# Totoketchup/Adaptive-MultiSpeaker-Separation

Hardware: AMD Instinct MI355X
Metric: mixtures/sec training throughput (2-spk, 256-filter adapt+BLSTM-DPCL) (higher is better)
Workload: dtype f32 (storage, accumulation and results f32; dense products issued on the 16-bit matrix pipe as fp16x3 / bf16x6 emulation of the f32 product -- `value_native_f32` is the same step on v_mfma_f32_32x32x2_f32)

## Files before the change

### adaptive-multispeaker-separation_amd/ams_hip/_lib.py

```python
import ctypes
import os
import re

_HERE = os.path.dirname(os.path.abspath(__file__))
LIB_PATH = os.environ.get('AMS_HIP_LIB') or os.path.join(_HERE, 'libams_hip.so')
HEADER_PATH = os.path.normpath(os.path.join(_HERE, '..', '..', 'include', 'ams.h'))

ABI_VERSION = 5

_CT = {
    'int': ctypes.c_int, 'long': ctypes.c_long, 'float': ctypes.c_float, 'size_t': ctypes.c_size_t,
    'int32_t': ctypes.c_int32, 'ams_status': ctypes.c_int32, 'void': None,
}


def parse_header(path=HEADER_PATH):
    src = open(path).read()
    src = re.sub(r'/\*.*?\*/', ' ', src, flags=re.S)
    protos = {}
    for m in re.finditer(r'\b(ams_status|size_t|int|long|void)\s+(ams_\w+)\s*\(([^)]*)\)\s*;', src):
        ret, name, args = m.group(1), m.group(2), m.group(3).strip()
        argtypes = []
        if args and args != 'void':
            for a in args.split(','):
# ... 50 lines not shown
```

### adaptive-multispeaker-separation_amd/ams_hip/functional.py

```python
import torch
from torch.autograd import Function

from . import ops


def _c(t):
    return t if t.is_contiguous() else t.contiguous()


class _Overlap(object):

    def __init__(self):
        self.enabled = False
        self.stream = None
        self.n_cap = 0
        self.deferred = []
        self.on_ready = None

    def side(self):
        if self.stream is None:
            import os
            self.stream = torch.cuda.Stream(priority=int(os.environ.get('AMS_SIDE_PRIORITY', '0')))
        return self.stream

# ... 205 lines not shown
        return ops.dense_fwd(x, W, b, amax=ctx.amax)

    @staticmethod
    def backward(ctx, du):
        x, W = ctx.saved_tensors
        du2 = _c(du).view(-1, W.shape[1])
        x2 = x.reshape(-1, x.shape[-1])
        b = ctx.bias
        am_dx = am_dw = None
        if ctx.amax is not None:
            adu = ops.amax_of(du2)
            am_dx, am_dw = (adu, ctx.amax[1]), (ctx.amax[0], adu)
        if OVERLAP.usable(W, b) and ctx.needs_input_grad[1] and ctx.needs_input_grad[2]:
            dx = None
            if _DENSE_MODE == 0 and _ORDER >= 1 and ctx.needs_input_grad[0]:
                dx = ops.gemm(du2, W, transB=True, amax=am_dx).view(x.shape)
            s = OVERLAP.fork(x2, du2)
            Nw = W.shape[1]
            cuts = _dw_cuts(Nw) if (_DENSE_MODE == 0 and ctx.needs_input_grad[0] and W.grad.stride(0) == Nw) else [(0, Nw)]

            def piece(n0, n1):
                Wg = W.grad if (n0, n1) == (0, Nw) else W.grad[:, n0:n1]
                dus = du2 if (n0, n1) == (0, Nw) else du2[:, n0:n1]
                with OVERLAP.capped('dense', _DENSE_MODE == 0):
                    fused = ops.gemm_at_b_colsum(x2, dus, Wg, b.grad[n0:n1], accumulate=True, amax=am_dw, ldc=W.grad.stride(0))
                    if not fused:
                        ops.gemm(x2, dus, transA=True, out=Wg, accumulate=True, amax=am_dw, M=x2.shape[1], N=n1 - n0, K=x2.shape[0],
                                 lda=x2.stride(0), ldb=du2.stride(0), ldc=W.grad.stride(0))
                if not fused:
                    ops.colsum_into(_c(dus), b.grad[n0:n1], True)
            with torch.cuda.stream(s):
                piece(*cuts[0])
            for i, c in enumerate(cuts[1:]):
                last = i == len(cuts) - 2
                OVERLAP.defer(lambda c=c, last=last: (piece(*c), OVERLAP.ready(W, b) if last else None))
            if len(cuts) == 1:
                OVERLAP.ready(W, b)
            if _DENSE_MODE == 2 and ctx.needs_input_grad[0]:
                torch.cuda.current_stream().wait_stream(s)
            if dx is None and ctx.needs_input_grad[0]:
                dx = ops.gemm(du2, W, transB=True, amax=am_dx).view(x.shape)
            return dx, None, None
        dx = ops.gemm(du2, W, transB=True, amax=am_dx).view(x.shape) if ctx.needs_input_grad[0] else None
        dW = ops.gemm(x2, du2, transA=True, amax=am_dw) if ctx.needs_input_grad[1] else None
        db = ops.colsum(du2) if ctx.needs_input_grad[2] else None
        return dx, dW, db


class L2Norm(Function):

    @staticmethod
    def forward(ctx, u, E):
        v, inv = ops.l2norm_fwd(u, E)
        ctx.save_for_backward(v, inv)
        ctx.E = E
        return v.view(u.shape[:-1] + (u.shape[-1] // E, E))

    @staticmethod
# ... 637 lines not shown
```

### adaptive-multispeaker-separation_amd/ams_hip/ops.py

```python
import ctypes
import os as _os

import torch

from ._lib import load, check, AmsError

_vp = ctypes.c_void_p


def _p(t):
    return _vp(t.data_ptr()) if t is not None else _vp(0)


def _s():
    return _vp(torch.cuda.current_stream().cuda_stream)


def _chk(*ts):
    for t in ts:
        if t is None:
            continue
        if not t.is_cuda:
            raise AmsError('ams_hip ops need device tensors (there is no CPU fallback)')
        if t.dtype != torch.float32 or not t.is_contiguous():
# ... 186 lines not shown
        a = getattr(b, '_ams_amax', None)
        if a is not None and a[1] == b._version:
            return a[0]
        b = b._base
    return absmax(t)


PASS = [0]


def _frozen(*ts):
    return all(getattr(t, '_ams_frozen', False) for t in ts)


def drop_frozen_derivatives(t):
    for k in ('_ams_amax_cache', '_ams_wcat', '_ams_wcat_amax', '_ams_kbound', '_ams_bcat', '_ams_ps_w'):
        if hasattr(t, k):
            delattr(t, k)


class _ParamSource(object):
    __slots__ = ('flat', 'bound', 'seen', 'event', 'used', 'next', 'rolled', '__weakref__')

    def __init__(self, flat):
        self.flat = flat
        self.bound = torch.zeros(1, dtype=torch.float32, device=flat.device)
        self.next = torch.zeros(192, dtype=torch.int32, device=flat.device)
        self.rolled = False
        self.seen = -1
        self.event = None
        self.used = -1
# ... 388 lines not shown
            and (bias is None or bias.data_ptr() % 16 == 0) and max(M, N) * ((K + 31) // 32 * 128) < 2 ** 31
            and load().ams_gemm_get_arith() != 0)


def forward_product(x2, W2, bias, out, amax, label, owner, ldc=None):
    M, K = x2.shape
    N = W2.shape[1]
    ldc = (out.stride(0) if out.dim() == 2 else N) if ldc is None else ldc
    if not (forward_product_presplit(M, N, K, out, bias, amax, label, ldc) and x2.stride(1) == 1 and W2.stride(1) == 1):
        return gemm(x2, W2, bias=bias, out=out, M=M, N=N, K=K, lda=x2.stride(0), ldb=W2.stride(0), ldc=ldc, label=label, amax=amax)
    a_img = ps_pack_rows(x2, amax[0])
    b_img = _ps_weight_image(W2, amax[1], owner)
    return gemm_ps(a_img, b_img, K, amax, bias=bias, out=out, ldc=ldc, label=label)


def gemm_at_b_colsum(A, B, out, bsum, accumulate=True, amax=None, ldc=None):
    K, M = A.shape
    N = B.shape[1]
    ldc = out.stride(0) if ldc is None else ldc
    ok = (M % 4 == 0 and N % 4 == 0 and A.stride(0) % 4 == 0 and B.stride(0) % 4 == 0 and A.stride(1) == 1 and B.stride(1) == 1
          and out.stride(-1) == 1 and bsum.stride(-1) == 1 and bsum.data_ptr() % 16 == 0
          and all(t.data_ptr() % 16 == 0 for t in (A, B)) and _os.environ.get('AMS_GEMM_NOVEC') is None)
    if not ok:
        return False
    lib = load()
    pad = LDS_PAD[0]
    nb = lib.ams_gemm_workspace_bytes(M, N, K, 1, pad)
    ws = _ws(nb, A) if nb else None
    bws = _ws(32 * N * 4, A)
    ev = PROFILE.begin() if PROFILE.enabled else None
# ... 266 lines not shown
    dx = None
    if need_dx:
        dxf = gemm(dZ, Kf, transB=True, M=M, N=D, K=4 * H, lda=8 * H, ldb=ldu, ldc=D,
                   out=torch.empty((M, D), dtype=torch.float32, device=x.device))
        dxb = gemm(dZ[4 * H:], Kb, transB=True, M=M, N=D, K=4 * H, lda=8 * H, ldb=ldu, ldc=D,
                   out=torch.empty((M, D), dtype=torch.float32, device=x.device))
        dx = dxf.view(B, T, D) * masks['in'][0] + dxb.view(B, T, D) * masks['in'][1]
    return dx, dKf, dbf, dKb, dbb


def blstm_bwd_dx(G, Kf, Kb, B, T, D, amax=None):
    H = Kf.shape[1] // 4
    M = B * T
    Wcat = blstm_wcat(Kf, Kb, D)
    dx = torch.empty((B, T, D), dtype=torch.float32, device=G.device)
    gemm(G.view(-1), Wcat, transB=True, out=dx, M=M, N=D, K=8 * H, lda=8 * H, ldb=8 * H, ldc=D, amax=amax)
    return dx


def blstm_bwd_weights(x, out, G, dKf, dbf, dKb, dbb, accumulate, part='all', dbpart=None, amax=None):
    lib = load()
    am_wx = (amax[0], amax[2]) if amax is not None else None
    am_u = (amax[1], amax[2]) if amax is not None else None
    B, T, D = x.shape
    H = dKf.shape[1] // 4
    M = B * T
    x2 = x.view(M, D)
    dZf = G.view(-1)
    dZb = G.view(-1)[4 * H:]
    acc = bool(accumulate)
    _chk_rows(dKf, dKb)
# ... 648 lines not shown
```

### adaptive-multispeaker-separation_amd/csrc/common.h

```cpp
#pragma once
#include <hip/hip_runtime.h>
#include <stdint.h>
#include <stddef.h>
#include "../../include/ams.h"

typedef float f32x4 __attribute__((ext_vector_type(4)));
typedef float f32x16 __attribute__((ext_vector_type(16)));

extern thread_local int g_ams_last_hip_error;

static inline ams_status ams_check_launch() {
    hipError_t e = hipGetLastError();
    if (e != hipSuccess) {
        g_ams_last_hip_error = (int)e;
        return AMS_E_LAUNCH_FAILED;
    }
    return AMS_OK;
}

#define AMS_REQUIRE(cond)            \
    do {                             \
        if (!(cond)) return AMS_E_INVALID_ARG; \
    } while (0)

static inline int ceil_div(long a, long b) { return (int)((a + b - 1) / b); }

namespace ams_detail {
size_t conv_maxpool_ps_bytes(int Bt, int L, int W, int N);
bool conv_maxpool_ps_applies(int Bt, int L, int W, int N);
ams_status conv_maxpool_ps(const float* x, const float* f, float* pmax, int32_t* pidx, int Bt, int L, int W, int N, int pl,
                           const float* amax_x, const float* amax_f, void* img, hipStream_t st);
}

__device__ __forceinline__ float wave_sum(float v) {
#pragma unroll
    for (int o = 32; o > 0; o >>= 1) v += __shfl_xor(v, o, 64);
    return v;
}
template <int S>
__device__ __forceinline__ float lane_above(float v) {
    const unsigned b = __builtin_bit_cast(unsigned, v);
    if constexpr (S == 32 || S == 16) {
        unsigned hi = b, lo = 0u;
        if constexpr (S == 32) asm volatile("s_nop 1\n\tv_permlane32_swap_b32 %0, %1\n\ts_nop 1" : "+v"(hi), "+v"(lo));
        else asm volatile("s_nop 1\n\tv_permlane16_swap_b32 %0, %1\n\ts_nop 1" : "+v"(hi), "+v"(lo));
        return __builtin_bit_cast(float, lo);
// ... 25 lines not shown
```

### adaptive-multispeaker-separation_amd/csrc/gemm.hip

```cpp
#include "common.h"
#include <stdlib.h>
#include <atomic>
#include <type_traits>

namespace {

struct LaunchOpt { const float* amax_a = nullptr; const float* amax_b = nullptr; int lds_pad = 0; void* sk_scratch = nullptr; size_t sk_bytes = 0;
                   unsigned* amax_out = nullptr; int force_cfg = -1; };
constexpr size_t AMS_SK_FLAG_BYTES = 8192;
constexpr size_t AMS_SK_SLOT_BYTES = (128 * 256 + 256) * sizeof(float);
std::atomic<int> g_gemm_arith{-1};

struct GemmTuning { int group_m, splits, x6cfg, x6rule, x6persist, sk; bool noprio, novec, f16x3; double x6waste; bool c_vec; };
inline const GemmTuning& tuning() {
    static const GemmTuning t = [] {
        GemmTuning v{0, 0, -1, 2, 1, 1, false, false, true, 1.30, true};
        if (const char* f = getenv("AMS_GEMM_CVEC")) v.c_vec = atoi(f) != 0;
        if (const char* f = getenv("AMS_GEMM_SK")) v.sk = atoi(f);
        if (const char* f = getenv("AMS_GEMM_X6WASTE")) v.x6waste = atof(f);
        if (const char* f = getenv("AMS_GEMM_GROUP_M")) v.group_m = atoi(f);
        if (const char* f = getenv("AMS_GEMM_SPLITS")) v.splits = atoi(f);
        v.noprio = getenv("AMS_GEMM_NOPRIO") != nullptr;
        { const char* e = getenv("AMS_X6_PERSIST"); v.x6persist = e ? atoi(e) : 1; }
        { const char* e = getenv("AMS_GEMM_F16X3"); v.f16x3 = !(e && atoi(e) == 0); }
// ... 1361 lines not shown
            if (blocks > 2048) blocks = 2048;
            hipLaunchKernelGGL(splitk_reduce_kernel, dim3(blocks, nbatch), dim3(256), 0, st, g.partial, g.C, g.bias, g.M, g.N, g.ldc,
                               splits, g.accumulate, g.c_zs, g.bias_zs);
        }
        s = ams_check_launch();
    }
    if (s == AMS_OK && bsum_out && !bsum_in_launch) {
        if (!vec || BMODE != B_ROW) return AMS_E_INVALID_ARG;
        hipLaunchKernelGGL(bsum_finish_kernel, dim3(ceil_div(g.N, 256)), dim3(256), 0, st, bsum_ws, bsum_out, g.N, splits, bsum_accumulate);
        s = ams_check_launch();
    }
    return s;
}

inline bool aligned16(const void* p) { return ((uintptr_t)p & 15) == 0; }

}

extern "C" {

void ams_gemm_set_arith(int mode) { g_gemm_arith.store(mode ? 1 : 0, std::memory_order_relaxed); }
int ams_gemm_get_arith(void) { return use_x6() ? 1 : 0; }

size_t ams_gemm_sk_scratch_bytes(void) {
    const size_t g8 = (size_t)(device_cus() + 7) / 8 * 8;
    const size_t a = g8 * 2 * (128 * 128 + 128) * sizeof(float), b = g8 * AMS_SK_SLOT_BYTES;
    return AMS_SK_FLAG_BYTES + (a > b ? a : b);
}

size_t ams_gemm_workspace_bytes(int M, int N, int K, int nbatch, int lds_pad) {
// ... 625 lines not shown
```

### adaptive-multispeaker-separation_amd/csrc/gemm_ps.hip

```cpp
#include "common.h"
#include <type_traits>

namespace {

typedef _Float16 f16x8_t __attribute__((ext_vector_type(8)));
typedef _Float16 f16x2_t __attribute__((ext_vector_type(2)));
typedef float f32x2_t __attribute__((ext_vector_type(2)));
typedef __attribute__((address_space(3))) void lds_void;
typedef int i32x4_t __attribute__((ext_vector_type(4)));

constexpr int PS_BK = 32, PS_BM = 128, PS_BN = 256, PS_NT = 512;
constexpr int PS_A_BYTES = PS_BM * 128, PS_B_BYTES = PS_BN * 128, PS_STAGE = PS_A_BYTES + PS_B_BYTES;
constexpr int PS_STAGES = 3;
constexpr int PS_BIAS_OFF = PS_STAGES * PS_STAGE;
constexpr int PS_LDS = PS_BIAS_OFF + 2 * 1024;

__device__ __forceinline__ unsigned ps_pk_f16(float a, float b) {
    const f32x2_t v = {a, b};
    return __builtin_bit_cast(unsigned, __builtin_convertvector(v, f16x2_t));
}
__device__ __forceinline__ void ps_split2(float a, float b, unsigned& hi, unsigned& lo) {
    hi = ps_pk_f16(a, b);
    const f16x2_t h = __builtin_bit_cast(f16x2_t, hi);
    lo = ps_pk_f16(a - (float)h[0], b - (float)h[1]);
// ... 90 lines not shown
    ps_split2(v[6] * s, v[7] * s, hi.w, lo.w);
    unsigned char* p = img + (((long)c * R + sgn) * lpp + t) * 32;
    *reinterpret_cast<uint4*>(p) = hi;
    *reinterpret_cast<uint4*>(p + 16) = lo;
}

struct PsArgs {
    const unsigned char* A; const unsigned char* B; float* C; const float* bias;
    const float* amax_a; const float* amax_b;
    int M, N, K;
    long ldc;
    unsigned pitch_a, pitch_b;
    int tiles_m, tiles_n, group_m;
    int conv_L, conv_R; unsigned conv_lpp; long a_bytes;
    int32_t* pidx;
};

__device__ __forceinline__ void ps_locate(const PsArgs& g, int item, int& tile_m, int& tile_n) {
    const int items = g.tiles_m * g.tiles_n;
    const int q = items / 8, r = items % 8, xcd = item % 8, idx = item / 8;
    const int bid = (xcd < r ? xcd * (q + 1) : r * (q + 1) + (xcd - r) * q) + idx;
    const int gm = g.group_m > 0 ? g.group_m : 1;
    const int band = bid / (gm * g.tiles_n), within = bid - band * (gm * g.tiles_n);
    const int band_rows = min(gm, g.tiles_m - band * gm);
    tile_n = within / band_rows;
    tile_m = band * gm + (within - tile_n * band_rows);
}

#ifndef AMS_PS_SLEEP
#define AMS_PS_SLEEP 0
#endif
#ifndef AMS_PS_STAMP
#define AMS_PS_STAMP 0
#endif
#if AMS_PS_STAMP
__device__ long long g_ps_stamp[1024 * 8 * 8];
#define PS_STAMP(ph) do { if (threadIdx.x == 0 && wi < 8) g_ps_stamp[((int)blockIdx.x * 8 + wi) * 8 + (ph)] = wall_clock64(); } while (0)
#else
#define PS_STAMP(ph) do { } while (0)
#endif

template <bool CONV>
__global__ __launch_bounds__(PS_NT, 1) void gemm_ps_kernel(const PsArgs g) {
    extern __shared__ __attribute__((aligned(1024))) unsigned char ps_smem[];
    const int tid = threadIdx.x, lane = tid & 63;
    const int wave = __builtin_amdgcn_readfirstlane(tid >> 6);
    const int wm = wave >> 2, wn = wave & 3;
    const int l31 = lane & 31, lk = lane >> 5;
    const int nk = (g.K + PS_BK - 1) / PS_BK;
    const int n_items = g.tiles_m * g.tiles_n, G = (int)gridDim.x;
    const int n_work = (n_items - (int)blockIdx.x + G - 1) / G;
    if (n_work <= 0) return;
    __builtin_amdgcn_s_setprio(2);

    auto rsrc = [](const unsigned char* p, long bytes) {
        const unsigned long long a = (unsigned long long)(uintptr_t)p;
        i32x4_t r = {(int)(unsigned)a, (int)(unsigned)((a >> 32) & 0xffffu), (int)bytes, 0x00020000};
        r.x = __builtin_amdgcn_readfirstlane(r.x); r.y = __builtin_amdgcn_readfirstlane(r.y);
        r.z = __builtin_amdgcn_readfirstlane(r.z); r.w = __builtin_amdgcn_readfirstlane(r.w);
        return r;
    };
    const i32x4_t rsA = rsrc(g.A, CONV ? g.a_bytes : (long)g.M * g.pitch_a), rsB = rsrc(g.B, (long)g.N * g.pitch_b);
    const i32x4_t rsBias = rsrc(reinterpret_cast<const unsigned char*>(g.bias), g.bias ? (long)g.N * 4 : 0);

    const int drow = lane >> 3, dslot = lane & 7;
    const int f_even = (drow >> 1) & 7, f_odd = (4 + (drow >> 1)) & 7;
    const unsigned pa_even = (unsigned)(dslot ^ f_even) * 16u, pa_odd = (unsigned)(dslot ^ f_odd) * 16u;
    unsigned voffA[2], voffB[4];

    const int ff = (l31 >> 1) & 7;
    unsigned fa[2], fb[2];
#pragma unroll
    for (int i = 0; i < 2; ++i) {
        if constexpr (CONV)
            fa[i] = (unsigned)((wm * 64 + 8 * (l31 & 7) + 4 * i + (l31 >> 3)) * 128 + ((lk ^ (l31 & 7)) * 16));
        else
            fa[i] = (unsigned)(((wm * 2 + i) * 32 + l31) * 128 + ((lk ^ ff) * 16));
    }
#pragma unroll
    for (int j = 0; j < 2; ++j) fb[j] = (unsigned)(PS_A_BYTES + ((wn * 2 + j) * 32 + l31) * 128 + ((lk ^ ff) * 16));

    const float sc_inv = (1.0f / ps_scale(g.amax_a[0])) * (1.0f / ps_scale(g.amax_b[0]));

    int tile_m, tile_n, m0, n0;
    auto setup = [&](int i) {
        ps_locate(g, (int)blockIdx.x + i * G, tile_m, tile_n);
        m0 = tile_m * PS_BM; n0 = tile_n * PS_BN;
        if constexpr (CONV) {
            const int sgn = m0 / g.conv_L, pb = m0 - sgn * g.conv_L;
#pragma unroll
            for (int q = 0; q < 2; ++q) {
                const int A_ = 2 * wave + q, a = A_ & 7, row = (A_ >> 3) * 64 + 8 * drow + a;
                const int p = pb + row;
                const unsigned pc = (unsigned)(dslot ^ a);
                const unsigned off = ((((unsigned)a * (unsigned)g.conv_R + (unsigned)sgn) * g.conv_lpp + (unsigned)(p >> 3) + (pc & 3u)) * 2u + (pc >> 2)) * 16u;
                voffA[q] = (m0 + row < g.M) ? off : 0xfffffff0u;
            }
        } else {
#pragma unroll
            for (int q = 0; q < 2; ++q) voffA[q] = (unsigned)(m0 + (2 * wave + q) * 8 + drow) * g.pitch_a + (q ? pa_odd : pa_even);
        }
#pragma unroll
        for (int q = 0; q < 4; ++q) voffB[q] = (unsigned)(n0 + (4 * wave + q) * 8 + drow) * g.pitch_b + ((q & 1) ? pa_odd : pa_even);
    };
    const unsigned lds0 = (unsigned)(uintptr_t)(lds_void*)ps_smem;
    auto issue1 = [&](int kt, int stage, int q) {
        const bool isA = q < 2;
        const unsigned ld = lds0 + (unsigned)(stage * PS_STAGE + (isA ? (2 * wave + q) * 1024 : PS_A_BYTES + (4 * wave + q - 2) * 1024));
        const unsigned vo = isA ? voffA[q] : voffB[q - 2];
        const int ko = kt * 128;
        unsigned keep;
        if (isA)
            asm volatile("s_mov_b32 %0, m0\n\ts_mov_b32 m0, %1\n\ts_nop 0\n\tbuffer_load_dwordx4 %2, %3, %4 offen lds\n\ts_mov_b32 m0, %0"
                         : "=&s"(keep) : "s"(ld), "v"(vo), "s"(rsA), "s"(ko) : "memory");
        else
            asm volatile("s_mov_b32 %0, m0\n\ts_mov_b32 m0, %1\n\ts_nop 0\n\tbuffer_load_dwordx4 %2, %3, %4 offen lds\n\ts_mov_b32 m0, %0"
                         : "=&s"(keep) : "s"(ld), "v"(vo), "s"(rsB), "s"(ko) : "memory");
    };
    auto issue = [&](int kt, int stage) {
#pragma unroll
        for (int q = 0; q < 6; ++q) issue1(kt, stage, q);
    };

    auto issue_bias = [&](int par) {
        if (wave == 0) {
            const unsigned lb = lds0 + (unsigned)(PS_BIAS_OFF + par * 1024);
            const unsigned vo = (unsigned)(n0 * 4 + lane * 16);
            unsigned keep;
            asm volatile("s_mov_b32 %0, m0\n\ts_mov_b32 m0, %1\n\ts_nop 0\n\tbuffer_load_dwordx4 %2, %3, 0 offen lds\n\ts_mov_b32 m0, %0"
                         : "=&s"(keep) : "s"(lb), "v"(vo), "s"(rsBias) : "memory");
        }
    };

    f32x16 acc[2][2], accs[2][2];
    f16x8_t carry[2][2];
    bool prime = true;
    auto frags = [&](const unsigned char* sb, int ks, f16x8_t (&a)[2][2], f16x8_t (&b)[2][2]) {
#pragma unroll
        for (int i = 0; i < 2; ++i)
#pragma unroll
// ... 3 lines not shown
            }
#pragma unroll
        for (int j = 0; j < 2; ++j)
#pragma unroll
            for (int p = 0; p < 2; ++p) b[j][p] = *reinterpret_cast<const f16x8_t*>(sb + (fb[j] ^ (unsigned)(ks * 32 + p * 64)));
    };
    auto four = [&](f32x16 (&c)[2][2], const f16x8_t (&a)[2][2], const f16x8_t (&b)[2][2], int pa, int pb) {
#pragma unroll
        for (int i = 0; i < 2; ++i)
#pragma unroll
            for (int j = 0; j < 2; ++j) c[i][j] = __builtin_amdgcn_mfma_f32_32x32x16_f16(a[i][pa], b[j][pb], c[i][j], 0, 0, 0);
#if AMS_PS_SLEEP
        __builtin_amdgcn_s_sleep(AMS_PS_SLEEP);
#endif
    };
    auto mfma_tile = [&](int stage, auto PRE, int kt2, int stage2) {
        constexpr bool pre = decltype(PRE)::value;
        const unsigned char* const sb = ps_smem + stage * PS_STAGE;
        f16x8_t a0[2][2], b0[2][2], a1[2][2], b1[2][2];
        if constexpr (CONV) {
            if (prime) {
#pragma unroll
                for (int ks = 0; ks < 2; ++ks)
#pragma unroll
                    for (int p = 0; p < 2; ++p) carry[ks][p] = *reinterpret_cast<const f16x8_t*>(sb + (fa[0] ^ (unsigned)(ks * 32 + p * 64)));
                prime = false;
            }
        }
        frags(sb, 0, a0, b0);
        __builtin_amdgcn_sched_barrier(0);
        four(accs, a0, b0, 1, 0);
        __builtin_amdgcn_sched_barrier(0);
        if constexpr (pre) issue1(kt2, stage2, 0);
        frags(sb, 1, a1, b1);
        __builtin_amdgcn_sched_barrier(0);
        four(accs, a0, b0, 0, 1);
        __builtin_amdgcn_sched_barrier(0);
        if constexpr (pre) issue1(kt2, stage2, 1);
        __builtin_amdgcn_sched_barrier(0);
        four(acc, a0, b0, 0, 0);
        __builtin_amdgcn_sched_barrier(0);
        if constexpr (pre) issue1(kt2, stage2, 2);
        __builtin_amdgcn_sched_barrier(0);
        four(accs, a1, b1, 1, 0);
        __builtin_amdgcn_sched_barrier(0);
        if constexpr (pre) issue1(kt2, stage2, 3);
        __builtin_amdgcn_sched_barrier(0);
        four(accs, a1, b1, 0, 1);
        __builtin_amdgcn_sched_barrier(0);
        if constexpr (pre) { issue1(kt2, stage2, 4); issue1(kt2, stage2, 5); }
        __builtin_amdgcn_sched_barrier(0);
        four(acc, a1, b1, 0, 0);
        if constexpr (CONV) {
#pragma unroll
            for (int p = 0; p < 2; ++p) { carry[0][p] = a0[1][p]; carry[1][p] = a1[1][p]; }
        }
    };

    setup(0);
    issue(0, 0);
    issue_bias(0);
    if (nk > 1) issue(1, 1);
    for (int wi = 0; wi < n_work; ++wi) {
        PS_STAMP(0);
#pragma unroll
        for (int i = 0; i < 2; ++i)
#pragma unroll
            for (int j = 0; j < 2; ++j)
#pragma unroll
                for (int r = 0; r < 16; ++r) { acc[i][j][r] = 0.f; accs[i][j][r] = 0.f; }
        prime = true;
        int st = 0;
        for (int kt = 0; kt < nk - 2; ++kt) {
            asm volatile("s_waitcnt vmcnt(6)" ::: "memory");
            __builtin_amdgcn_s_barrier();
            mfma_tile(st, std::true_type{}, kt + 2, st == 0 ? 2 : st - 1);
            st = st == 2 ? 0 : st + 1;
        }
        if (nk >= 2) {
            asm volatile("s_waitcnt vmcnt(6)" ::: "memory");
            __builtin_amdgcn_s_barrier();
            mfma_tile(st, std::false_type{}, 0, 0);
            st = st == 2 ? 0 : st + 1;
        }
        asm volatile("s_waitcnt vmcnt(0)" ::: "memory");
        __builtin_amdgcn_s_barrier();
        mfma_tile(st, std::false_type{}, 0, 0);
        PS_STAMP(1);
        const int em0 = m0, en0 = n0;
        const bool more = wi + 1 < n_work;
        asm volatile("s_waitcnt lgkmcnt(0)" ::: "memory");
        __builtin_amdgcn_s_barrier();
        if (more) {
            setup(wi + 1);
            issue(0, 0);
            issue_bias((wi + 1) & 1);
        }
        if constexpr (CONV) {
            float* const sred = reinterpret_cast<float*>(ps_smem + PS_STAGE);
            int* const srow = reinterpret_cast<int*>(sred + 256);
#pragma unroll
            for (int j = 0; j < 2; ++j) {
                float best = -3.4e38f;
                int brow = 0x7fffffff;
#pragma unroll
                for (int i = 0; i < 2; ++i) {
                    const f32x16 c = (acc[i][j] + accs[i][j]) * sc_inv;
#pragma unroll
// ... 15 lines not shown
                    if (ob2 > best || (ob2 == best && or2 < brow)) { best = ob2; brow = or2; }
                    const int col = en0 + wn * 64 + j * 32 + l31;
                    if (col < g.N) { g.C[(long)(em0 / PS_BM) * g.N + col] = best; g.pidx[(long)(em0 / PS_BM) * g.N + col] = brow; }
                }
                asm volatile("s_waitcnt lgkmcnt(0)" ::: "memory");
                __builtin_amdgcn_s_barrier();
            }
            PS_STAMP(2);
            if (more && nk > 1) issue(1, 1);
            continue;
        }
        float* const wl = reinterpret_cast<float*>(ps_smem + PS_STAGE) + wave * 2048;
        const int rr = lane >> 4, c4 = (lane & 15) * 4;
        const int col = en0 + wn * 64 + c4;
        const bool cok = col < g.N;
        const float4 bv = *reinterpret_cast<const float4*>(ps_smem + PS_BIAS_OFF + (wi & 1) * 1024 + (wn * 64 + c4) * 4);
#pragma unroll
        for (int i = 0; i < 2; ++i) {
#pragma unroll
            for (int j = 0; j < 2; ++j) {
                acc[i][j] = (acc[i][j] + accs[i][j]) * sc_inv;
#pragma unroll
                for (int r = 0; r < 16; ++r) wl[((r & 3) + 8 * (r >> 2) + 4 * lk) * 64 + j * 32 + l31] = acc[i][j][r];
            }
#pragma unroll
            for (int p8 = 0; p8 < 8; ++p8) {
                const int rl = p8 * 4 + rr;
                float4 v = *reinterpret_cast<const float4*>(wl + rl * 64 + c4);
                const int row = em0 + (wm * 2 + i) * 32 + rl;
                if (row < g.M && cok) {
                    v.x += bv.x; v.y += bv.y; v.z += bv.z; v.w += bv.w;
                    *reinterpret_cast<float4*>(g.C + (long)row * g.ldc + col) = v;
                }
            }
        }
        PS_STAMP(2);
        if (more) {
            asm volatile("s_waitcnt lgkmcnt(0)" ::: "memory");
            __builtin_amdgcn_s_barrier();
            if (nk > 1) issue(1, 1);
        }
    }
}

inline int ps_group_m(int tiles_m, int tiles_n) {
    int gm = 8;
    if (gm > tiles_m) gm = tiles_m;
    (void)tiles_n;
    return gm < 1 ? 1 : gm;
}

}

extern "C" {

// ... 23 lines not shown
    PsArgs g{};
    g.A = (const unsigned char*)A_img; g.B = (const unsigned char*)B_img; g.C = C; g.bias = bias; g.amax_a = amax_a; g.amax_b = amax_b;
    g.M = M; g.N = N; g.K = K; g.ldc = ldc;
    g.pitch_a = g.pitch_b = (unsigned)ams_ps_image_pitch(K);
    AMS_REQUIRE((long)M * g.pitch_a < (1L << 31) && (long)N * g.pitch_b < (1L << 31));
    g.tiles_m = (M + PS_BM - 1) / PS_BM; g.tiles_n = (N + PS_BN - 1) / PS_BN;
    g.group_m = ps_group_m(g.tiles_m, g.tiles_n);
    static const int cus = [] { int dev = 0, n = 0; if (hipGetDevice(&dev) != hipSuccess || hipDeviceGetAttribute(&n, hipDeviceAttributeMultiprocessorCount, dev) != hipSuccess || n <= 0) n = 256; return n; }();
    static const bool raised = [] { return hipFuncSetAttribute((const void*)gemm_ps_kernel<false>, hipFuncAttributeMaxDynamicSharedMemorySize, PS_LDS) == hipSuccess; }();
    if (!raised) return AMS_E_LAUNCH_FAILED;
    const int items = g.tiles_m * g.tiles_n;
    int grid = items < cus ? items : cus;
    if (grid >= 8) grid -= grid % 8;
    hipLaunchKernelGGL(gemm_ps_kernel<false>, dim3((unsigned)grid), dim3(PS_NT), PS_LDS, (hipStream_t)stream, g);
    return ams_check_launch();
}

}

namespace ams_detail {

static inline unsigned conv_lpp(int L, int W) { return (unsigned)((L - 1) / 8 + 4 * ((W + 31) / 32) + 1); }

__attribute__((visibility("hidden"))) size_t conv_maxpool_ps_bytes(int Bt, int L, int W, int N) {
    const size_t a = (size_t)8 * 2 * Bt * conv_lpp(L, W) * 16, b = ams_ps_image_bytes(N, W);
    return (a + 255) / 256 * 256 + (b + 255) / 256 * 256;
}
__attribute__((visibility("hidden"))) bool conv_maxpool_ps_applies(int Bt, int L, int W, int N) {
    return L % PS_BM == 0 && N % 4 == 0 && (size_t)8 * 2 * Bt * conv_lpp(L, W) * 16 < ((size_t)1 << 31) - 64 && ams_ps_image_bytes(N, W) < ((size_t)1 << 31);
}
// ... 31 lines not shown
```

### include/ams.h

```cpp
#ifndef AMS_H
#define AMS_H
#include <stddef.h>
#include <stdint.h>

#ifdef __cplusplus
extern "C" {
#endif

#define AMS_ABI_VERSION 5

typedef int32_t ams_status;
#define AMS_OK 0
#define AMS_E_INVALID_ARG (-1)
#define AMS_E_WORKSPACE_TOO_SMALL (-2)
#define AMS_E_LAUNCH_FAILED (-3)

int ams_last_error(void);
int ams_abi_version(void);

ams_status ams_front_filter_fwd(const float* w, const float* bases, float* f, int W, int N, void* stream);
ams_status ams_front_filter_bwd(const float* w, const float* bases, const float* df, float* dw, float* dbases, int W, int N,
                                void* stream);

size_t ams_front_conv_fwd_workspace_bytes(int Bt, int L, int W, int N, int hop);
// ... 20 lines not shown
                                     int T, int S, void* stream);

size_t ams_gemm_workspace_bytes(int M, int N, int K, int nbatch, int lds_pad);
size_t ams_gemm_sk_scratch_bytes(void);
void ams_gemm_set_arith(int mode);
int ams_gemm_get_arith(void);
ams_status ams_gemm_f32(int transA, int transB, int M, int N, int K, const float* A, long lda, const float* B, long ldb, float* C,
                        long ldc, const float* bias, int accumulate, int mask_period, int mask_skip, const float* amax_a,
                        const float* amax_b, int lds_pad, void* ws, size_t ws_bytes, void* sk_scratch, size_t sk_bytes, void* stream);
size_t ams_ps_image_pitch(int K);
size_t ams_ps_image_bytes(int rows, int K);
ams_status ams_ps_pack_rows(const float* x, long ldx, void* img, int R, int K, const float* amax, void* stream);
ams_status ams_ps_pack_cols(const float* w, long ldw, void* img, int K, int N, const float* amax, void* stream);
ams_status ams_gemm_ps(int M, int N, int K, const void* A_img, const void* B_img, float* C, long ldc, const float* bias,
                       const float* amax_a, const float* amax_b, void* stream);

ams_status ams_gemm_f32_at_b_colsum(int M, int N, int K, const float* A, long lda, const float* B, long ldb, float* C, long ldc,
                                    int accumulate, float* bsum_out, int bsum_accumulate, float* bsum_ws, const float* amax_a,
                                    const float* amax_b, int lds_pad, void* ws, size_t ws_bytes, void* sk_scratch, size_t sk_bytes,
                                    void* stream);
ams_status ams_gemm_f32_batched(int transA, int transB, int M, int N, int K, const float* A, long lda, long a_zs, const float* B,
                                long ldb, long b_zs, float* C, long ldc, long c_zs, int nbatch, int accumulate, int mask_period,
                                int mask_skip, const float* amax_a, const float* amax_b, int lds_pad, void* ws, size_t ws_bytes,
                                void* sk_scratch, size_t sk_bytes, void* stream);
ams_status ams_range_share(const float* x, long rows, long cols, long ld, const float* bound, float* out3, void* stream);
ams_status ams_absmax_f32(const float* x, long n, float* out, void* stream);

ams_status ams_make_masks(const float* rep_non_mix, float* Y, int32_t* argmax, int B, int S, long TF, float a, float b,
                          int take_abs, void* stream);

// ... 146 lines not shown
```

Measured before the change: 23330.

## Route backward dx products through pre-split fp16 kernel with in-kernel A splitting

```diff
diff --git a/adaptive-multispeaker-separation_amd/ams_hip/_lib.py b/adaptive-multispeaker-separation_amd/ams_hip/_lib.py
--- a/adaptive-multispeaker-separation_amd/ams_hip/_lib.py
+++ b/adaptive-multispeaker-separation_amd/ams_hip/_lib.py
@@ -6,7 +6,7 @@
 LIB_PATH = os.environ.get('AMS_HIP_LIB') or os.path.join(_HERE, 'libams_hip.so')
 HEADER_PATH = os.path.normpath(os.path.join(_HERE, '..', '..', 'include', 'ams.h'))
 
-ABI_VERSION = 5
+ABI_VERSION = 6
 
 _CT = {
     'int': ctypes.c_int, 'long': ctypes.c_long, 'float': ctypes.c_float, 'size_t': ctypes.c_size_t,
diff --git a/adaptive-multispeaker-separation_amd/ams_hip/functional.py b/adaptive-multispeaker-separation_amd/ams_hip/functional.py
--- a/adaptive-multispeaker-separation_amd/ams_hip/functional.py
+++ b/adaptive-multispeaker-separation_amd/ams_hip/functional.py
@@ -243,7 +243,7 @@
         if OVERLAP.usable(W, b) and ctx.needs_input_grad[1] and ctx.needs_input_grad[2]:
             dx = None
             if _DENSE_MODE == 0 and _ORDER >= 1 and ctx.needs_input_grad[0]:
-                dx = ops.gemm(du2, W, transB=True, amax=am_dx).view(x.shape)
+                dx = ops.backward_product(du2, W, am_dx, W).view(x.shape)
             s = OVERLAP.fork(x2, du2)
             Nw = W.shape[1]
             cuts = _dw_cuts(Nw) if (_DENSE_MODE == 0 and ctx.needs_input_grad[0] and W.grad.stride(0) == Nw) else [(0, Nw)]
@@ -268,9 +268,9 @@
             if _DENSE_MODE == 2 and ctx.needs_input_grad[0]:
                 torch.cuda.current_stream().wait_stream(s)
             if dx is None and ctx.needs_input_grad[0]:
-                dx = ops.gemm(du2, W, transB=True, amax=am_dx).view(x.shape)
+                dx = ops.backward_product(du2, W, am_dx, W).view(x.shape)
             return dx, None, None
-        dx = ops.gemm(du2, W, transB=True, amax=am_dx).view(x.shape) if ctx.needs_input_grad[0] else None
+        dx = ops.backward_product(du2, W, am_dx, W).view(x.shape) if ctx.needs_input_grad[0] else None
         dW = ops.gemm(x2, du2, transA=True, amax=am_dw) if ctx.needs_input_grad[1] else None
         db = ops.colsum(du2) if ctx.needs_input_grad[2] else None
         return dx, dW, db
diff --git a/adaptive-multispeaker-separation_amd/ams_hip/ops.py b/adaptive-multispeaker-separation_amd/ams_hip/ops.py
--- a/adaptive-multispeaker-separation_amd/ams_hip/ops.py
+++ b/adaptive-multispeaker-separation_amd/ams_hip/ops.py
@@ -224,7 +224,7 @@
 
 
 def drop_frozen_derivatives(t):
-    for k in ('_ams_amax_cache', '_ams_wcat', '_ams_wcat_amax', '_ams_kbound', '_ams_bcat', '_ams_ps_w'):
+    for k in ('_ams_amax_cache', '_ams_wcat', '_ams_wcat_amax', '_ams_kbound', '_ams_bcat', '_ams_ps_w', '_ams_ps_dx'):
         if hasattr(t, k):
             delattr(t, k)
 
@@ -643,6 +643,47 @@
     return gemm_ps(a_img, b_img, K, amax, bias=bias, out=out, ldc=ldc, label=label)
 
 
+DX_PS = _os.environ.get('AMS_GEMM_DX_PS', '1') != '0'
+
+
+def _ps_dx_weight_image(W2, amax_w, owner):
+    c = getattr(owner, '_ams_ps_dx', None)
+    if (c is not None and c[1] == W2.data_ptr() and c[2] == tuple(W2.shape) and c[3] is amax_w and (c[0] == PASS[0] or _frozen(owner))):
+        return c[4]
+    img = ps_pack_rows(W2, amax_w)
+    owner._ams_ps_dx = (PASS[0], W2.data_ptr(), tuple(W2.shape), amax_w, img)
+    return img
+
+
+def backward_product(dU2, W2, amax, owner, out=None, label=''):
+    M, K = dU2.shape
+    N = W2.shape[0]
+    if out is None:
+        out = torch.empty((M, N), dtype=torch.float32, device=dU2.device)
+    ldc = out.stride(0) if out.dim() == 2 else N
+    lda = dU2.stride(0)
+    key = ('gemm', label, M, N, K, False, True)
+    lib = load()
+    if not (DX_PS and F16X3 and amax is not None and amax[0] is not None and amax[1] is not None and key not in F16_AUDIT.denied
+            and not F16_AUDIT.active and LDS_PAD[0] == 0 and N % 4 == 0 and ldc % 4 == 0 and lda % 4 == 0 and dU2.stride(1) == 1
+            and W2.stride(1) == 1 and out.data_ptr() % 16 == 0 and dU2.data_ptr() % 16 == 0 and M * lda * 4 < 2 ** 31
+            and N * ((K + 31) // 32 * 128) < 2 ** 31 and lib.ams_gemm_get_arith() != 0
+            and K % 4 == 0 and (N + 255) // 256 * 256 <= 1.30 * N):
+        return gemm(dU2, W2, transB=True, out=out, M=M, N=N, K=K, lda=lda, ldb=W2.stride(0), ldc=ldc, label=label, amax=amax)
+    b_img = _ps_dx_weight_image(W2, amax[1], owner)
+    nb = lib.ams_gemm_ps_a_workspace_bytes(M, N, K)
+    ws = _ws(nb, dU2) if nb else None
+    ev = PROFILE.begin() if PROFILE.enabled else None
+    cur = torch.cuda.current_stream()
+    amax[0].record_stream(cur)
+    amax[1].record_stream(cur)
+    check(lib.ams_gemm_ps_a_f32(M, N, K, _p(dU2), lda, _p(b_img), _p(out), ldc, _p(amax[0]), _p(amax[1]), _p(ws), nb, _s()),
+          'ams_gemm_ps_a_f32')
+    if ev is not None:
+        PROFILE.end(ev, 2.0 * M * N * K, 4.0 * (M * K + K * N + M * N), 'gemm16ps_a<0,1>', label)
+    return out
+
+
 def gemm_at_b_colsum(A, B, out, bsum, accumulate=True, amax=None, ldc=None):
     K, M = A.shape
     N = B.shape[1]
@@ -939,7 +980,7 @@
     M = B * T
     Wcat = blstm_wcat(Kf, Kb, D)
     dx = torch.empty((B, T, D), dtype=torch.float32, device=G.device)
-    gemm(G.view(-1), Wcat, transB=True, out=dx, M=M, N=D, K=8 * H, lda=8 * H, ldb=8 * H, ldc=D, amax=amax)
+    backward_product(G.view(M, 8 * H), Wcat, amax, Kf, out=dx.view(M, D))
     return dx
 
 
diff --git a/adaptive-multispeaker-separation_amd/csrc/common.h b/adaptive-multispeaker-separation_amd/csrc/common.h
--- a/adaptive-multispeaker-separation_amd/csrc/common.h
+++ b/adaptive-multispeaker-separation_amd/csrc/common.h
@@ -30,6 +30,8 @@
 bool conv_maxpool_ps_applies(int Bt, int L, int W, int N);
 ams_status conv_maxpool_ps(const float* x, const float* f, float* pmax, int32_t* pidx, int Bt, int L, int W, int N, int pl,
                            const float* amax_x, const float* amax_f, void* img, hipStream_t st);
+int dx_splits(int M, int N, int K, size_t ws_bytes, int* kps);
+ams_status splitk_reduce(const float* partial, float* C, int M, int N, long ldc, int splits, hipStream_t st);
 }
 
 __device__ __forceinline__ float wave_sum(float v) {
diff --git a/adaptive-multispeaker-separation_amd/csrc/gemm.hip b/adaptive-multispeaker-separation_amd/csrc/gemm.hip
--- a/adaptive-multispeaker-separation_amd/csrc/gemm.hip
+++ b/adaptive-multispeaker-separation_amd/csrc/gemm.hip
@@ -1399,6 +1399,28 @@
 }
 
 inline bool aligned16(const void* p) { return ((uintptr_t)p & 15) == 0; }
+
+}
+
+namespace ams_detail {
+
+__attribute__((visibility("hidden"))) int dx_splits(int M, int N, int K, size_t ws_bytes, int* kps) {
+    int splits = choose_splits(M, N, K, 1, x6_plan(3));
+    if (tuning().splits > 0) splits = tuning().splits;
+    while (splits > 1 && (size_t)splits * M * N * sizeof(float) > ws_bytes) --splits;
+    int k = ceil_div(ceil_div(K, splits), X6_BK) * X6_BK;
+    *kps = k;
+    return ceil_div(K, k);
+}
+
+__attribute__((visibility("hidden"))) ams_status splitk_reduce(const float* partial, float* C, int M, int N, long ldc, int splits, hipStream_t st) {
+    const long total = (long)M * N;
+    if (N % 4 || ldc % 4 || (((uintptr_t)C | (uintptr_t)partial) & 15) || total >= (1L << 31)) return AMS_E_INVALID_ARG;
+    int blocks = (int)((total / 4 + 255) / 256);
+    if (blocks > 4096) blocks = 4096;
+    hipLaunchKernelGGL(splitk_reduce_vec_kernel, dim3(blocks, 1), dim3(256), 0, st, partial, C, (const float*)nullptr, M, N, ldc, splits, 0, 0L, 0L);
+    return ams_check_launch();
+}
 
 }
 
diff --git a/adaptive-multispeaker-separation_amd/csrc/gemm_ps.hip b/adaptive-multispeaker-separation_amd/csrc/gemm_ps.hip
--- a/adaptive-multispeaker-separation_amd/csrc/gemm_ps.hip
+++ b/adaptive-multispeaker-separation_amd/csrc/gemm_ps.hip
@@ -128,12 +128,18 @@
     int tiles_m, tiles_n, group_m;
     int conv_L, conv_R; unsigned conv_lpp; long a_bytes;
     int32_t* pidx;
+    const float* Af; long lda;
+    int splits, kps;
+    float* partial;
 };
 
-__device__ __forceinline__ void ps_locate(const PsArgs& g, int item, int& tile_m, int& tile_n) {
-    const int items = g.tiles_m * g.tiles_n;
+template <bool AF32 = false>
+__device__ __forceinline__ void ps_locate(const PsArgs& g, int item, int& tile_m, int& tile_n, int& split) {
+    const int ntiles = g.tiles_m * g.tiles_n, items = AF32 ? ntiles * g.splits : ntiles;
     const int q = items / 8, r = items % 8, xcd = item % 8, idx = item / 8;
-    const int bid = (xcd < r ? xcd * (q + 1) : r * (q + 1) + (xcd - r) * q) + idx;
+    int bid = (xcd < r ? xcd * (q + 1) : r * (q + 1) + (xcd - r) * q) + idx;
+    split = 0;
+    if constexpr (AF32) { split = bid / ntiles; bid -= split * ntiles; }
     const int gm = g.group_m > 0 ? g.group_m : 1;
     const int band = bid / (gm * g.tiles_n), within = bid - band * (gm * g.tiles_n);
     const int band_rows = min(gm, g.tiles_m - band * gm);
@@ -154,15 +160,16 @@
 #define PS_STAMP(ph) do { } while (0)
 #endif
 
-template <bool CONV>
+template <bool CONV, bool AF32 = false>
 __global__ __launch_bounds__(PS_NT, 1) void gemm_ps_kernel(const PsArgs g) {
+    static_assert(!(CONV && AF32), "one A operand form per instance");
     extern __shared__ __attribute__((aligned(1024))) unsigned char ps_smem[];
     const int tid = threadIdx.x, lane = tid & 63;
     const int wave = __builtin_amdgcn_readfirstlane(tid >> 6);
     const int wm = wave >> 2, wn = wave & 3;
     const int l31 = lane & 31, lk = lane >> 5;
-    const int nk = (g.K + PS_BK - 1) / PS_BK;
-    const int n_items = g.tiles_m * g.tiles_n, G = (int)gridDim.x;
+    int nk = (g.K + PS_BK - 1) / PS_BK;
+    const int n_items = g.tiles_m * g.tiles_n * (AF32 ? g.splits : 1), G = (int)gridDim.x;
     const int n_work = (n_items - (int)blockIdx.x + G - 1) / G;
     if (n_work <= 0) return;
     __builtin_amdgcn_s_setprio(2);
@@ -174,7 +181,8 @@
         r.z = __builtin_amdgcn_readfirstlane(r.z); r.w = __builtin_amdgcn_readfirstlane(r.w);
         return r;
     };
-    const i32x4_t rsA = rsrc(g.A, CONV ? g.a_bytes : (long)g.M * g.pitch_a), rsB = rsrc(g.B, (long)g.N * g.pitch_b);
+    const i32x4_t rsA = AF32 ? rsrc(reinterpret_cast<const unsigned char*>(g.Af), (long)g.M * g.lda * 4)
+                             : rsrc(g.A, CONV ? g.a_bytes : (long)g.M * g.pitch_a), rsB = rsrc(g.B, (long)g.N * g.pitch_b);
     const i32x4_t rsBias = rsrc(reinterpret_cast<const unsigned char*>(g.bias), g.bias ? (long)g.N * 4 : 0);
 
     const int drow = lane >> 3, dslot = lane & 7;
@@ -196,11 +204,19 @@
 
     const float sc_inv = (1.0f / ps_scale(g.amax_a[0])) * (1.0f / ps_scale(g.amax_b[0]));
 
-    int tile_m, tile_n, m0, n0;
+    int tile_m, tile_n, m0, n0, split = 0, kt0 = 0, kend = g.K;
+    const int ar = tid >> 2, ag = tid & 3, af = (ar >> 1) & 7;
+    unsigned avoff = 0;
+    f32x4 ra0 = {}, ra1 = {};
     auto setup = [&](int i) {
-        ps_locate(g, (int)blockIdx.x + i * G, tile_m, tile_n);
+        ps_locate<AF32>(g, (int)blockIdx.x + i * G, tile_m, tile_n, split);
         m0 = tile_m * PS_BM; n0 = tile_n * PS_BN;
-        if constexpr (CONV) {
+        if constexpr (AF32) {
+            kt0 = split * (g.kps / PS_BK);
+            kend = min(g.K, (split + 1) * g.kps);
+            nk = (kend - kt0 * PS_BK + PS_BK - 1) / PS_BK;
+            avoff = (m0 + ar < g.M) ? (unsigned)((long)(m0 + ar) * g.lda * 4) + (unsigned)ag * 32u : 0x80000000u;
+        } else if constexpr (CONV) {
             const int sgn = m0 / g.conv_L, pb = m0 - sgn * g.conv_L;
 #pragma unroll
             for (int q = 0; q < 2; ++q) {
@@ -222,7 +238,7 @@
         const bool isA = q < 2;
         const unsigned ld = lds0 + (unsigned)(stage * PS_STAGE + (isA ? (2 * wave + q) * 1024 : PS_A_BYTES + (4 * wave + q - 2) * 1024));
         const unsigned vo = isA ? voffA[q] : voffB[q - 2];
-        const int ko = kt * 128;
+        const int ko = (kt0 + kt) * 128;
         unsigned keep;
         if (isA)
             asm volatile("s_mov_b32 %0, m0\n\ts_mov_b32 m0, %1\n\ts_nop 0\n\tbuffer_load_dwordx4 %2, %3, %4 offen lds\n\ts_mov_b32 m0, %0"
@@ -233,11 +249,33 @@
     };
     auto issue = [&](int kt, int stage) {
 #pragma unroll
-        for (int q = 0; q < 6; ++q) issue1(kt, stage, q);
+        for (int q = AF32 ? 2 : 0; q < 6; ++q) issue1(kt, stage, q);
+    };
+    auto load_a = [&](int kt) {
+        const unsigned vo = avoff + (unsigned)((kt0 + kt) * 128);
+        asm volatile("s_nop 4\n\tbuffer_load_dwordx4 %0, %2, %3, 0 offen\n\tbuffer_load_dwordx4 %1, %2, %3, 0 offen offset:16"
+                     : "=&v"(ra0), "=&v"(ra1) : "v"(vo), "s"(rsA) : "memory");
+    };
+    const float sc_a = AF32 ? ps_scale(g.amax_a[0]) : 1.0f;
+    auto cut_a = [&](int kt, int stage) {
+        float v[8] = {ra0[0], ra0[1], ra0[2], ra0[3], ra1[0], ra1[1], ra1[2], ra1[3]};
+        const int kb = (kt0 + kt) * PS_BK;
+        if (kb + PS_BK > kend) {
+#pragma unroll
+            for (int j = 0; j < 8; ++j) v[j] = (kb + ag * 8 + j < kend) ? v[j] : 0.f;
+        }
+        uint4 hi, lo;
+        ps_split2(v[0] * sc_a, v[1] * sc_a, hi.x, lo.x);
+        ps_split2(v[2] * sc_a, v[3] * sc_a, hi.y, lo.y);
+        ps_split2(v[4] * sc_a, v[5] * sc_a, hi.z, lo.z);
+        ps_split2(v[6] * sc_a, v[7] * sc_a, hi.w, lo.w);
+        unsigned char* const p = ps_smem + stage * PS_STAGE + ar * 128;
+        *reinterpret_cast<uint4*>(p + ((ag ^ af) * 16)) = hi;
+        *reinterpret_cast<uint4*>(p + (((4 + ag) ^ af) * 16)) = lo;
     };
 
     auto issue_bias = [&](int par) {
-        if (wave == 0) {
+        if (!AF32 && wave == 0) {
             const unsigned lb = lds0 + (unsigned)(PS_BIAS_OFF + par * 1024);
             const unsigned vo = (unsigned)(n0 * 4 + lane * 16);
             unsigned keep;
@@ -271,8 +309,8 @@
         __builtin_amdgcn_s_sleep(AMS_PS_SLEEP);
 #endif
     };
-    auto mfma_tile = [&](int stage, auto PRE, int kt2, int stage2) {
-        constexpr bool pre = decltype(PRE)::value;
+    auto mfma_tile = [&](int stage, auto PRE, int kt2, int stage2, auto CUT, int stage_c) {
+        constexpr bool pre = decltype(PRE)::value, cut = decltype(CUT)::value;
         const unsigned char* const sb = ps_smem + stage * PS_STAGE;
         f16x8_t a0[2][2], b0[2][2], a1[2][2], b1[2][2];
         if constexpr (CONV) {
@@ -288,12 +326,15 @@
         __builtin_amdgcn_sched_barrier(0);
         four(accs, a0, b0, 1, 0);
         __builtin_amdgcn_sched_barrier(0);
-        if constexpr (pre) issue1(kt2, stage2, 0);
+        if constexpr (AF32) {
+            if constexpr (cut) cut_a(kt2 - 1, stage_c);
+            if constexpr (pre) load_a(kt2);
+        } else if constexpr (pre) issue1(kt2, stage2, 0);
         frags(sb, 1, a1, b1);
         __builtin_amdgcn_sched_barrier(0);
         four(accs, a0, b0, 0, 1);
         __builtin_amdgcn_sched_barrier(0);
-        if constexpr (pre) issue1(kt2, stage2, 1);
+        if constexpr (pre && !AF32) issue1(kt2, stage2, 1);
         __builtin_amdgcn_sched_barrier(0);
         four(acc, a0, b0, 0, 0);
         __builtin_amdgcn_sched_barrier(0);
@@ -314,10 +355,20 @@
         }
     };
 
+    auto start_af32 = [&]() {
+        load_a(0);
+        asm volatile("s_waitcnt vmcnt(0)" : "+v"(ra0), "+v"(ra1) :: "memory");
+        cut_a(0, 0);
+        issue(0, 0);
+        if (nk > 1) { load_a(1); issue(1, 1); }
+    };
     setup(0);
-    issue(0, 0);
-    issue_bias(0);
-    if (nk > 1) issue(1, 1);
+    if constexpr (AF32) start_af32();
+    else {
+        issue(0, 0);
+        issue_bias(0);
+        if (nk > 1) issue(1, 1);
+    }
     for (int wi = 0; wi < n_work; ++wi) {
         PS_STAMP(0);
 #pragma unroll
@@ -329,26 +380,29 @@
         prime = true;
         int st = 0;
         for (int kt = 0; kt < nk - 2; ++kt) {
-            asm volatile("s_waitcnt vmcnt(6)" ::: "memory");
+            if constexpr (AF32) asm volatile("s_waitcnt vmcnt(4) lgkmcnt(0)" : "+v"(ra0), "+v"(ra1) :: "memory");
+            else asm volatile("s_waitcnt vmcnt(6)" ::: "memory");
             __builtin_amdgcn_s_barrier();
-            mfma_tile(st, std::true_type{}, kt + 2, st == 0 ? 2 : st - 1);
+            mfma_tile(st, std::true_type{}, kt + 2, st == 0 ? 2 : st - 1, std::true_type{}, st == 2 ? 0 : st + 1);
             st = st == 2 ? 0 : st + 1;
         }
         if (nk >= 2) {
-            asm volatile("s_waitcnt vmcnt(6)" ::: "memory");
+            if constexpr (AF32) asm volatile("s_waitcnt vmcnt(4) lgkmcnt(0)" : "+v"(ra0), "+v"(ra1) :: "memory");
+            else asm volatile("s_waitcnt vmcnt(6)" ::: "memory");
             __builtin_amdgcn_s_barrier();
-            mfma_tile(st, std::false_type{}, 0, 0);
+            mfma_tile(st, std::false_type{}, nk, 0, std::true_type{}, st == 2 ? 0 : st + 1);
             st = st == 2 ? 0 : st + 1;
         }
-        asm volatile("s_waitcnt vmcnt(0)" ::: "memory");
+        if constexpr (AF32) asm volatile("s_waitcnt vmcnt(0) lgkmcnt(0)" ::: "memory");
+        else asm volatile("s_waitcnt vmcnt(0)" ::: "memory");
         __builtin_amdgcn_s_barrier();
-        mfma_tile(st, std::false_type{}, 0, 0);
+        mfma_tile(st, std::false_type{}, 0, 0, std::false_type{}, 0);
         PS_STAMP(1);
         const int em0 = m0, en0 = n0;
         const bool more = wi + 1 < n_work;
         asm volatile("s_waitcnt lgkmcnt(0)" ::: "memory");
         __builtin_amdgcn_s_barrier();
-        if (more) {
+        if (more && !AF32) {
             setup(wi + 1);
             issue(0, 0);
             issue_bias((wi + 1) & 1);
@@ -394,7 +448,9 @@
         const int rr = lane >> 4, c4 = (lane & 15) * 4;
         const int col = en0 + wn * 64 + c4;
         const bool cok = col < g.N;
-        const float4 bv = *reinterpret_cast<const float4*>(ps_smem + PS_BIAS_OFF + (wi & 1) * 1024 + (wn * 64 + c4) * 4);
+        const float4 bv = AF32 ? float4{0.f, 0.f, 0.f, 0.f} : *reinterpret_cast<const float4*>(ps_smem + PS_BIAS_OFF + (wi & 1) * 1024 + (wn * 64 + c4) * 4);
+        float* const out = (AF32 && g.splits > 1) ? g.partial + (long)split * g.M * g.N : g.C;
+        const long ldo = (AF32 && g.splits > 1) ? (long)g.N : g.ldc;
 #pragma unroll
         for (int i = 0; i < 2; ++i) {
 #pragma unroll
@@ -409,8 +465,8 @@
                 float4 v = *reinterpret_cast<const float4*>(wl + rl * 64 + c4);
                 const int row = em0 + (wm * 2 + i) * 32 + rl;
                 if (row < g.M && cok) {
-                    v.x += bv.x; v.y += bv.y; v.z += bv.z; v.w += bv.w;
-                    *reinterpret_cast<float4*>(g.C + (long)row * g.ldc + col) = v;
+                    if constexpr (!AF32) { v.x += bv.x; v.y += bv.y; v.z += bv.z; v.w += bv.w; }
+                    *reinterpret_cast<float4*>(out + (long)row * ldo + col) = v;
                 }
             }
         }
@@ -418,7 +474,8 @@
         if (more) {
             asm volatile("s_waitcnt lgkmcnt(0)" ::: "memory");
             __builtin_amdgcn_s_barrier();
-            if (nk > 1) issue(1, 1);
+            if constexpr (AF32) { setup(wi + 1); start_af32(); }
+            else if (nk > 1) issue(1, 1);
         }
     }
 }
@@ -472,6 +529,39 @@
     if (grid >= 8) grid -= grid % 8;
     hipLaunchKernelGGL(gemm_ps_kernel<false>, dim3((unsigned)grid), dim3(PS_NT), PS_LDS, (hipStream_t)stream, g);
     return ams_check_launch();
+}
+
+size_t ams_gemm_ps_a_workspace_bytes(int M, int N, int K) {
+    if (M <= 0 || N <= 0 || K <= 0) return 0;
+    int kps = 0;
+    const int splits = ams_detail::dx_splits(M, N, K, ~(size_t)0, &kps);
+    return splits > 1 ? (size_t)splits * M * N * sizeof(float) : 0;
+}
+
+ams_status ams_gemm_ps_a_f32(int M, int N, int K, const float* A, long lda, const void* B_img, float* C, long ldc, const float* amax_a,
+                             const float* amax_b, void* ws, size_t ws_bytes, void* stream) {
+    AMS_REQUIRE(A && B_img && C && amax_a && amax_b && M > 0 && N > 0 && K > 0 && lda >= K);
+    AMS_REQUIRE(N % 4 == 0 && ldc % 4 == 0 && ldc >= N && lda % 4 == 0 &&
+                ((((uintptr_t)C) | ((uintptr_t)A) | ((uintptr_t)B_img) | ((uintptr_t)ws)) & 15) == 0);
+    PsArgs g{};
+    g.Af = A; g.lda = lda; g.B = (const unsigned char*)B_img; g.C = C; g.bias = nullptr; g.amax_a = amax_a; g.amax_b = amax_b;
+    g.M = M; g.N = N; g.K = K; g.ldc = ldc;
+    g.pitch_b = (unsigned)ams_ps_image_pitch(K);
+    AMS_REQUIRE((long)M * lda * 4 < (1L << 31) && (long)N * g.pitch_b < (1L << 31));
+    g.splits = ams_detail::dx_splits(M, N, K, ws ? ws_bytes : 0, &g.kps);
+    g.partial = (float*)ws;
+    g.tiles_m = (M + PS_BM - 1) / PS_BM; g.tiles_n = (N + PS_BN - 1) / PS_BN;
+    g.group_m = ps_group_m(g.tiles_m, g.tiles_n);
+    static const int cus = [] { int dev = 0, n = 0; if (hipGetDevice(&dev) != hipSuccess || hipDeviceGetAttribute(&n, hipDeviceAttributeMultiprocessorCount, dev) != hipSuccess || n <= 0) n = 256; return n; }();
+    static const bool raised = [] { return hipFuncSetAttribute((const void*)gemm_ps_kernel<false, true>, hipFuncAttributeMaxDynamicSharedMemorySize, PS_LDS) == hipSuccess; }();
+    if (!raised) return AMS_E_LAUNCH_FAILED;
+    const int items = g.tiles_m * g.tiles_n * g.splits;
+    int grid = items < cus ? items : cus;
+    if (grid >= 8) grid -= grid % 8;
+    hipLaunchKernelGGL((gemm_ps_kernel<false, true>), dim3((unsigned)grid), dim3(PS_NT), PS_LDS, (hipStream_t)stream, g);
+    ams_status r = ams_check_launch();
+    if (r == AMS_OK && g.splits > 1) r = ams_detail::splitk_reduce(g.partial, C, M, N, ldc, g.splits, (hipStream_t)stream);
+    return r;
 }
 
 }
diff --git a/include/ams.h b/include/ams.h
--- a/include/ams.h
+++ b/include/ams.h
@@ -7,7 +7,7 @@
 extern "C" {
 #endif
 
-#define AMS_ABI_VERSION 5
+#define AMS_ABI_VERSION 6
 
 typedef int32_t ams_status;
 #define AMS_OK 0
@@ -58,6 +58,9 @@
 ams_status ams_ps_pack_cols(const float* w, long ldw, void* img, int K, int N, const float* amax, void* stream);
 ams_status ams_gemm_ps(int M, int N, int K, const void* A_img, const void* B_img, float* C, long ldc, const float* bias,
                        const float* amax_a, const float* amax_b, void* stream);
+size_t ams_gemm_ps_a_workspace_bytes(int M, int N, int K);
+ams_status ams_gemm_ps_a_f32(int M, int N, int K, const float* A, long lda, const void* B_img, float* C, long ldc, const float* amax_a,
+                             const float* amax_b, void* ws, size_t ws_bytes, void* stream);
 
 ams_status ams_gemm_f32_at_b_colsum(int M, int N, int K, const float* A, long lda, const float* B, long ldb, float* C, long ldc,
                                     int accumulate, float* bsum_out, int bsum_accumulate, float* bsum_ws, const float* amax_a,
```

New measurement: 24170 (median of 6 runs). 1.04x the previous value.
